# mdolab/dafoam

Hardware: NVIDIA H100
Metric: dRdWTPsi_GCells_per_s (higher is better)
Workload: dtype f64

## Files before the change

dafoam_b200/csrc/capi.cpp:

```cpp
#include "../../include/dab200.h"
#include "solver.hpp"
#include <cstring>
#include <string>

using namespace dab;

struct dab_solver
{
    Solver s;
};

static thread_local std::string g_err;
static dab_exchange_fn g_cbExchange = nullptr;
static dab_allreduce_fn g_cbAllreduce = nullptr;
static void* g_cbCtx = nullptr;

#define DAB_TRY try {
#define DAB_CATCH                                   \
    }                                               \
    catch (const std::exception& e)                 \
    {                                               \
        g_err = e.what();                           \
        return 1;                                   \
    }                                               \
// ... 587 lines not shown
        stats->pc_assemblies = s->s.kry.pcAssemblies;
        stats->n_matvec = st.nMatvec;
    }
    DAB_CATCH
}

int dab_solve_linear_eqn(dab_solver* s, const double* rhs, double* sol, int* fail, dab_ksp_stats* stats)
{
    DAB_TRY
    need(s, "solver");
    need(rhs, "rhs");
    need(sol, "sol");
    KspStats st;
    const int f = s->s.solveLinearEqn(rhs, sol, st);
    if (fail) *fail = f;
    if (stats)
    {
        stats->iterations = st.iterations;
        stats->converged_reason = st.reason;
        stats->initial_residual = st.r0;
        stats->final_residual = st.rn;
        stats->solve_seconds = st.solveSec;
        stats->pc_setup_seconds = st.pcSec;
        stats->pc_assemblies = s->s.kry.pcAssemblies;
        stats->n_matvec = st.nMatvec;
    }
    DAB_CATCH
}

int dab_calc_function(dab_solver* s, const char* name, double* value)
{
    DAB_TRY
    need(s, "solver");
    need(name, "name");
    need(value, "value");
    *value = s->s.calcFunction(name);
    DAB_CATCH
}

int dab_get_input_size(dab_solver* s, const char* name, const char* type, int64_t* out)
{
    DAB_TRY
    need(s, "solver");
    need(type, "type");
    (void)name;
    if (std::string(type) == "stateVar") *out = s->s.nDof();
    else if (std::string(type) == "patchVelocity") *out = 2;
    else if (std::string(type) == "volCoord") *out = (int64_t)s->s.hm.points.size();
    else if (std::string(type) == "patchVar") { need(name, "name"); *out = s->s.findPatchVar(name).nComp; }
    else if (std::string(type) == "fvSourcePar") { need(name, "name"); *out = (int64_t)s->s.findFvSourcePar(name).indices.size(); }
    else throw Error(std::string("getInputSize: unsupported input type ") + type);
    DAB_CATCH
}

int dab_get_output_size(dab_solver* s, const char* name, const char* type, int64_t* out)
{
    DAB_TRY
    need(s, "solver");
    need(type, "type");
    (void)name;
    const std::string t(type);
    if (t == "residual") *out = s->s.nDof();
    else if (t == "function") *out = 1;
    else throw Error("getOutputSize: unsupported output type " + t);
    DAB_CATCH
}

int dab_bench_set_vector(dab_solver* s, const double* x)
{
    DAB_TRY
    need(s, "solver");
    need(x, "x");
    s->s.be.h2d(s->s.dX.p, x, (size_t)s->s.nDof() * sizeof(double));
    DAB_CATCH
}

int dab_bench_device(dab_solver* s, int which, int n, double* ms_per_call, int64_t* kernel_launches)
{
    DAB_TRY
    need(s, "solver");
    need(ms_per_call, "ms_per_call");
    Solver& S = s->s;
    S.ensureRecorded();
    const long l0 = S.be.launches;
    auto t = S.be.timer();
    S.be.sync();
    t.start();
    for (int i = 0; i < n; i++)
    {
        switch (which)
        {
        case 0: S.matVecDev(S.dX.p, S.dY2.p); break;
        case 1: S.forward(0, S.dR.p); break;
        case 2: S.benchKernel(0); break;
        case 3: S.benchKernel(1); break;
        case 4: S.benchKernel(2); break;
        default: throw Error("dab_bench_device: unknown selector");
        }
    }
    *ms_per_call = t.stopMs() / (n > 0 ? n : 1);
    if (kernel_launches) *kernel_launches = S.be.launches - l0;
    DAB_CATCH
}

int dab_algorithmic_bytes(dab_solver* s, int which, int64_t* bytes)
{
    DAB_TRY
    need(s, "solver");
    need(bytes, "bytes");
    const HostMesh& m = s->s.hm;
    const int64_t nDof = s->s.nDof();
    const int64_t vecs = which == 0 ? 3 : 2;
    *bytes = 8 * vecs * nDof + (int64_t)m.nIF * (8 * 10 + 4 * 2) + (int64_t)m.nBF * (8 * 6 + 4 * 2) + (int64_t)m.nC * (8 * 5);
    DAB_CATCH
}

}
```

dafoam_b200/csrc/krylov.hpp:

```cpp
#pragma once
#include "backend.hpp"
#include "views.hpp"
#include "comm.hpp"
#include <atomic>
#include <cmath>
#include <thread>
#include <cstdint>
#include <vector>

namespace dab
{

struct KspStats
{
    int iterations = 0, reason = 0;
    double r0 = 0, rn = 0, solveSec = 0, pcSec = 0;
    int nMatvec = 0;
};

struct EllView
{
    int n;
    const int64_t* rowBase;
    const int32_t* rowStride;
// ... 55 lines not shown
        *q += eps * sc;
    }
};

struct FdFill
{
    EllView A;
    const int32_t* list;
    const int32_t* iperm;
    const int32_t* perm;
    const double *R0, *R1;
    double ieps;
    DAB_HD void operator()(int t) const
    {
        const int i = iperm[list[t]];
        const int64_t base = A.rowBase[i];
        const int64_t st = A.rowStride[i];
        const int len = A.rowLen[i];
        for (int e = 0; e < len; e++)
        {
            const int r = perm[A.col[base + e * st]];
            A.val[base + e * st] = (R1[r] - R0[r]) * ieps;
        }
    }
};

DAB_HD int ellFind(const EllView& A, int i, int j)
{
    const int64_t base = A.rowBase[i], st = A.rowStride[i];
    int lo = 0, hi = A.rowLen[i] - 1;
    while (lo <= hi)
    {
        const int mid = (lo + hi) >> 1;
        const int c = A.col[base + mid * st];
        if (c == j) return mid;
        if (c < j) lo = mid + 1;
        else hi = mid - 1;
    }
    return -1;
}

struct IluFactorColour
{
    EllView A;
    ColourView cv;
    double shift;
    DAB_HD void operator()(int t) const
    {
        for (int s = 0; s < cv.nSlots; s++)
        {
            if (t >= cv.slotCount[s]) break;
            const int i = cv.slotStart[s] + t;
            const int64_t bi = A.rowBase[i], si = A.rowStride[i];
            const int len = A.rowLen[i], di = A.diag[i];
            double rowMax = 0.0;
            for (int e = 0; e < len; e++)
            {
                const double v = fabs(A.val[bi + e * si]);
                rowMax = v > rowMax ? v : rowMax;
            }
            for (int e = 0; e < di; e++)
            {
                const int k = A.col[bi + e * si];
                const int64_t bk = A.rowBase[k], sk = A.rowStride[k];
                const int dk = A.diag[k], lk = A.rowLen[k];
                const double lik = A.val[bi + e * si] * A.val[bk + dk * sk];
                A.val[bi + e * si] = lik;
                if (lik == 0.0) continue;
                int pj = e + 1;
                for (int q = dk + 1; q < lk && pj < len; q++)
                {
                    const int j = A.col[bk + q * sk];
                    while (pj < len && A.col[bi + pj * si] < j) pj++;
                    if (pj < len && A.col[bi + pj * si] == j) A.val[bi + pj * si] -= lik * A.val[bk + q * sk];
                }
            }
            double d = A.val[bi + di * si];
            if (!(fabs(d) > shift * rowMax)) d = (d < 0.0 ? -1.0 : 1.0) * (rowMax > 0.0 ? shift * rowMax : 1.0);
            A.val[bi + di * si] = 1.0 / d;
        }
    }
};


template <int TRI_LANES>
DAB_HD double triRowDot(const EllView& A, int64_t bi, int64_t si, int e0, int e1, int lane, const double* y)
{
    double acc = 0.0;
    if (A.valF)
        for (int e = e0 + lane; e < e1; e += TRI_LANES) acc += (double)A.valF[bi + e * si] * y[A.col[bi + e * si]];
    else
        for (int e = e0 + lane; e < e1; e += TRI_LANES) acc += A.val[bi + e * si] * y[A.col[bi + e * si]];
    return acc;
}

template <int TRI_LANES>
struct TriLowerColour
{
    EllView A;
    ColourView cv;
    double* y;
    DAB_HD void operator()(int tt) const
    {
#if defined(__CUDA_ARCH__)
        const int t = tt / TRI_LANES, lane = tt - t * TRI_LANES;
        for (int s = 0; s < cv.nSlots; s++)
        {
            const bool on = t < cv.slotCount[s];
            const int i = cv.slotStart[s] + t;
            double acc = 0.0;
            if (on) acc = triRowDot<TRI_LANES>(A, cv.slotBase[s] + t, cv.slotCount[s], 0, A.diag[i], lane, y);
            for (int o = 1; o < TRI_LANES; o <<= 1) acc += __shfl_xor_sync(0xffffffffu, acc, o, TRI_LANES);
            if (on && lane == 0) y[i] -= acc;
            __syncwarp();
        }
#else
        if (tt % TRI_LANES) return;
        const int t = tt / TRI_LANES;
        for (int s = 0; s < cv.nSlots; s++)
        {
            if (t >= cv.slotCount[s]) break;
            const int i = cv.slotStart[s] + t;
            const int64_t bi = A.rowBase[i], si = A.rowStride[i];
            double part[TRI_LANES];
            for (int l = 0; l < TRI_LANES; l++) part[l] = triRowDot<TRI_LANES>(A, bi, si, 0, A.diag[i], l, y);
            for (int o = 1; o < TRI_LANES; o <<= 1)
                for (int l = 0; l < TRI_LANES; l++)
                    if (!(l & o)) part[l] += part[l | o];
            y[i] -= part[0];
        }
#endif
    }
};

template <int TRI_LANES>
struct TriUpperColour
{
    EllView A;
    ColourView cv;
    double* x;
    DAB_HD void operator()(int tt) const
    {
#if defined(__CUDA_ARCH__)
        const int t = tt / TRI_LANES, lane = tt - t * TRI_LANES;
        for (int s = cv.nSlots - 1; s >= 0; s--)
        {
            const bool on = t < cv.slotCount[s];
            const int i = cv.slotStart[s] + t;
            int64_t bi = 0, si = 0;
            int di = 0;
            double acc = 0.0;
            if (on)
            {
                bi = cv.slotBase[s] + t; si = cv.slotCount[s]; di = A.diag[i];
                acc = triRowDot<TRI_LANES>(A, bi, si, di + 1, A.rowLen[i], lane, x);
            }
            for (int o = 1; o < TRI_LANES; o <<= 1) acc += __shfl_xor_sync(0xffffffffu, acc, o, TRI_LANES);
            if (on && lane == 0) x[i] = (x[i] - acc) * (A.valF ? (double)A.valF[bi + di * si] : A.val[bi + di * si]);
            __syncwarp();
        }
#else
        if (tt % TRI_LANES) return;
        const int t = tt / TRI_LANES;
        for (int s = cv.nSlots - 1; s >= 0; s--)
        {
            if (t >= cv.slotCount[s]) continue;
            const int i = cv.slotStart[s] + t;
            const int64_t bi = A.rowBase[i], si = A.rowStride[i];
            const int di = A.diag[i];
            double part[TRI_LANES];
            for (int l = 0; l < TRI_LANES; l++) part[l] = triRowDot<TRI_LANES>(A, bi, si, di + 1, A.rowLen[i], l, x);
            for (int o = 1; o < TRI_LANES; o <<= 1)
                for (int l = 0; l < TRI_LANES; l++)
                    if (!(l & o)) part[l] += part[l | o];
            x[i] = (x[i] - part[0]) * (A.valF ? (double)A.valF[bi + di * si] : A.val[bi + di * si]);
        }
#endif
    }
};

DAB_HD double ellVal(const EllView& A, int64_t o) { return A.valF ? (double)A.valF[o] : A.val[o]; }

struct CvtToFloat
{
    const double* src;
    float* dst;
    DAB_HD void operator()(int i) const { dst[i] = (float)src[i]; }
};

struct GatherVec
{
    const double* src;
    const int32_t* idx;
    double* dst;
    DAB_HD void operator()(int i) const { dst[i] = src[idx[i]]; }
};
struct ScatterVec
{
    const double* src;
    const int32_t* idx;
    double* dst;
    DAB_HD void operator()(int i) const { dst[idx[i]] = src[i]; }
};
struct JacobiApply
{
    const double *src, *dinv;
    double* dst;
    DAB_HD void operator()(int i) const { dst[i] = src[i] * dinv[i]; }
};

struct MultiAxpy
{
    const double* V;
    int64_t ld;
    int k;
    const double* h;
    double* w;
    int assign;
    DAB_HD void operator()(int i) const
    {
        double s = 0.0;
        for (int j = 0; j < k; j++) s += h[j] * V[(int64_t)j * ld + i];
        w[i] = assign ? s : w[i] - s;
    }
};
struct ScaleCopy
{
    const double* src;
    double a;
    double* dst;
    DAB_HD void operator()(int i) const { dst[i] = a * src[i]; }
};
struct AxpyVec
{
    const double* x;
    double a;
    double* y;
    DAB_HD void operator()(int i) const { y[i] += a * x[i]; }
};
struct SubVec
{
    const double* b;
    double* r;
    DAB_HD void operator()(int i) const { r[i] = b[i] - r[i]; }
};

#ifndef DAB_HOSTSIM
constexpr int DOT_TILE = 8;
constexpr int DOT_BLOCKS = 132 * 4;
constexpr int DOT_THREADS = 256;
__global__ void __launch_bounds__(DOT_THREADS) multiDotPartial(const double* __restrict__ V, int64_t ld, int k, const double* __restrict__ w,
                                                               int n, double* __restrict__ partial)
{
    __shared__ double sm[DOT_THREADS / 32][DOT_TILE];
    const int lane = threadIdx.x & 31, warp = threadIdx.x >> 5;
    for (int j0 = 0; j0 < k; j0 += DOT_TILE)
    {
        const int nj = (k - j0) < DOT_TILE ? (k - j0) : DOT_TILE;
        double acc[DOT_TILE];
#pragma unroll
        for (int j = 0; j < DOT_TILE; j++) acc[j] = 0.0;
        for (int i = blockIdx.x * blockDim.x + threadIdx.x; i < n; i += gridDim.x * blockDim.x)
        {
            const double wi = w[i];
#pragma unroll
            for (int j = 0; j < DOT_TILE; j++)
                if (j < nj) acc[j] += V[(int64_t)(j0 + j) * ld + i] * wi;
        }
#pragma unroll
        for (int j = 0; j < DOT_TILE; j++)
        {
            double v = acc[j];
            for (int o = 16; o > 0; o >>= 1) v += __shfl_down_sync(0xffffffffu, v, o);
            if (lane == 0) sm[warp][j] = v;
        }
        __syncthreads();
        if (threadIdx.x < nj)
        {
            double v = 0.0;
            for (int q = 0; q < DOT_THREADS / 32; q++) v += sm[q][threadIdx.x];
            partial[(int64_t)blockIdx.x * k + j0 + threadIdx.x] = v;
        }
        __syncthreads();
    }
}
__global__ void multiDotFinal(const double* __restrict__ partial, int nb, int k, double* __restrict__ out)
// ... 382 lines not shown
```

dafoam_b200/csrc/launch_traits.hpp:

```cpp
#pragma once
#include "backend.hpp"
#include "fwd_kernels.hpp"
#include "rev_kernels.hpp"
#include "comp_kernels.hpp"
#include "comp_rev_kernels.hpp"
#include "primal_kernels.hpp"
#include "comp_primal_kernels.hpp"

namespace dab
{

#if !defined(DAB_HOSTSIM)
#ifndef DAB_REVB_MINBLOCKS
#define DAB_REVB_MINBLOCKS 2
#endif
#ifndef DAB_FWDB_MINBLOCKS
#define DAB_FWDB_MINBLOCKS 3
#endif
template <int NF, int FEAT> struct LaunchTraits<RevB<NF, FEAT>> { static constexpr int minBlocks = DAB_REVB_MINBLOCKS; };
template <int NF> struct LaunchTraits<RevA<NF>> { static constexpr int minBlocks = 5; };
template <int NF> struct LaunchTraits<RevC<NF>> { static constexpr int minBlocks = 4; };
template <int NF, int FEAT> struct LaunchTraits<FwdB<NF, FEAT>> { static constexpr int minBlocks = DAB_FWDB_MINBLOCKS; };
template <int NF, int FEAT> struct LaunchTraits<UEqnAssemble<NF, FEAT>> { static constexpr int minBlocks = DAB_FWDB_MINBLOCKS; };
template <int NF> struct LaunchTraits<NutEqnAssemble<NF>> { static constexpr int minBlocks = 4; };
template <int NF> struct LaunchTraits<cFwdB<NF>> { static constexpr int minBlocks = 2; };
template <int NF> struct LaunchTraits<cUEqnAssemble<NF>> { static constexpr int minBlocks = 2; };
template <int NF> struct LaunchTraits<cEEqnAssemble<NF>> { static constexpr int minBlocks = 3; };
template <int NF> struct LaunchTraits<cNutEqnAssemble<NF>> { static constexpr int minBlocks = 3; };
template <int NF> struct LaunchTraits<cPEqnAssemble<NF>> { static constexpr int minBlocks = 4; };
template <int NF> struct LaunchTraits<cPhiUpdate<NF>> { static constexpr int minBlocks = 4; };
#ifndef DAB_CREVA_MINBLOCKS
#define DAB_CREVA_MINBLOCKS 4
#endif
#ifndef DAB_CREVB_MINBLOCKS
#define DAB_CREVB_MINBLOCKS 3
#endif
#ifndef DAB_CREVE_MINBLOCKS
#define DAB_CREVE_MINBLOCKS 4
#endif
template <int NF> struct LaunchTraits<cRevB<NF>> { static constexpr int minBlocks = DAB_CREVB_MINBLOCKS; };
template <int NF> struct LaunchTraits<cRevA<NF>> { static constexpr int minBlocks = DAB_CREVA_MINBLOCKS; };
template <int NF> struct LaunchTraits<cRevE<NF>> { static constexpr int minBlocks = DAB_CREVE_MINBLOCKS; };
template <int NF> struct LaunchTraits<cRevC<NF>> { static constexpr int minBlocks = 4; };
template <int NF> struct LaunchTraits<cFwdE<NF>> { static constexpr int minBlocks = 4; };
template <int NF> struct LaunchTraits<cFwdC<NF>> { static constexpr int minBlocks = 4; };
#endif

}
```

dafoam_b200/csrc/solver.hpp:

```cpp
#pragma once
#include "backend.hpp"
#include "mesh.hpp"
#include "views.hpp"
#include "fwd_kernels.hpp"
#include "rev_kernels.hpp"
#include "tile_kernels.hpp"
#include "comp_kernels.hpp"
#include "comp_rev_kernels.hpp"
#include "krylov.hpp"
#include "primal_kernels.hpp"
#include "geom_kernels.hpp"
#include "comp_primal_kernels.hpp"
#include "launch_traits.hpp"
#include "partition.hpp"
#include "comm.hpp"
#include <chrono>
#include <cstdlib>
#include <cstdio>
#include <fstream>
#include <map>
#include <sys/stat.h>
#include <set>

namespace dab
// ... 2182 lines not shown
                    if (bj < 0) throw Error("writeSensMapSurface: no surface point within 9999999 of a wall point");
                    norm2 += best * best;
                    for (int k = 0; k < 3; k++) sens[(size_t)3 * (f - hm.nIF) + k] += dFdXs[3 * bj + k];
                }
                for (int k = 0; k < 3; k++) sens[(size_t)3 * (f - hm.nIF) + k] /= 3.0;
            }
        }
        const std::string dir = caseDirectory + "/" + timeName;
        ::mkdir(dir.c_str(), 0755);
        FILE* f = fopen((dir + "/" + name).c_str(), "w");
        if (!f) throw Error("cannot write " + dir + "/" + name);
        fprintf(f, "FoamFile\n{\n    version 2.0;\n    format ascii;\n    class volVectorField;\n    location \"%s\";\n    object %s;\n}\n\n"
                   "dimensions [0 0 0 0 0 0 0];\n\ninternalField uniform (0 0 0);\n\nboundaryField\n{\n", timeName.c_str(), name.c_str());
        for (size_t ip = 0; ip < hm.patches.size(); ip++)
        {
            const PatchDef& p = hm.patches[ip];
            fprintf(f, "    %s\n    {\n        type fixedValue;\n", p.name.c_str());
            if (hm.patchGeom[ip] == PG_WALL)
            {
                fprintf(f, "        value nonuniform List<vector> %d(", p.size);
                for (int i = 0; i < p.size; i++)
                {
                    const double* v = &sens[(size_t)3 * (p.start + i - hm.nIF)];
                    fprintf(f, "%s(%.17g %.17g %.17g)", i ? " " : "", v[0], v[1], v[2]);
                }
                fprintf(f, ");\n");
            }
            else
                fprintf(f, "        value uniform (0 0 0);\n");
            fprintf(f, "    }\n");
        }
        fprintf(f, "}\n");
        fclose(f);
        return std::sqrt(norm2);
    }

    void writeMeshPoints(const double* pts, const std::string& dirName) const
    {
        if (ghosted()) throw Error("mesh output needs an undecomposed mesh without cyclic patches in this build");
        const std::string d1 = caseDirectory + "/" + dirName, d2 = d1 + "/polyMesh";
        ::mkdir(d1.c_str(), 0755);
        ::mkdir(d2.c_str(), 0755);
        FILE* f = fopen((d2 + "/points").c_str(), "w");
        if (!f) throw Error("cannot write " + d2 + "/points");
        fprintf(f, "FoamFile\n{\n    version 2.0;\n    format ascii;\n    class vectorField;\n    location \"%s/polyMesh\";\n    object points;\n}\n\n%d\n(\n",
                dirName.c_str(), hm.nP);
        for (int i = 0; i < hm.nP; i++) fprintf(f, "(%.17g %.17g %.17g)\n", pts[3 * i], pts[3 * i + 1], pts[3 * i + 2]);
        fprintf(f, ")\n");
        fclose(f);
    }
    void readMeshPoints(const std::string& timeName)
    {
        std::vector<double> pts;
        readVectorField(caseDirectory + "/" + timeName + "/polyMesh/points", pts);
        if (pts.size() != hm.points.size()) throw Error("readMeshPoints: " + timeName + "/polyMesh/points has the wrong size");
        updateMesh(pts.data());
    }
    void readStateVars(const std::string& timeName) { initialStates(caseDirectory, timeName); }

    VolCoord volc;
    void uploadGeometry();
    void deviceGeometry();
    void downloadGeometry();
    void updateMesh(const double* pts);
    void volCoordSetup();
    void volCoordProduct(const double* psi, const FunctionDef* function, double seed, double* out);

    Primal primal;
    VecOps primalOps;
    void primalSetup();
    const double* primalSums(int k);
    void primalResidual(const EqnView& e, const double* x, const double* g, double* res);
    void primalJacobi(const EqnView& e, double* x, double* tmp, const double* g, const SegControl& ctl, double* res0);
    void primalCoarseSetup();
    void primalCoarseRefresh(const EqnView& e);
    void primalPrecond(const EqnView& e, const double* r, double* z);
    int primalPcg(const EqnView& e, double* x, const SegControl& ctl, double& res0);
    int solvePrimal(PrimalStats& st);

    void pcSymbolic();
    void calcPC();
    void applyPC(const double* v, double* z);
    void applyIlu(const double* v, double* z);
    void coarseSetup();
    void coarseRestrict(const double* v, bool toHost = true);
    int kspExtraMatvecs = 0;
    int solveLinearEqn(const double* rhs, double* sol, KspStats& st);
    int solveIdrs(const double* rhs, double* sol, KspStats& st);
    int solveFixedPoint(const double* rhs, double* sol, KspStats& st);
};

}

#include "solver_krylov.hpp"
#include "solver_primal.hpp"
#include "solver_volcoord.hpp"
```

dafoam_b200/csrc/solver_krylov.hpp:

```cpp
#pragma once
#include <algorithm>
#include <chrono>
#include <cstdio>

#include <memory>
#include <thread>

namespace dab
{

namespace detail
{
struct CellGraph
{
    int nC;
    std::vector<int> off, adj, stamp, queue;
    int tick = 0;
    void build(const HostMesh& m, const std::vector<int>* alias = nullptr)
    {
        nC = m.nC;
        auto cellOf = [&](int c) { return c < nC ? c : (alias ? (*alias)[c - nC] : -1); };
        off.assign(nC + 1, 0);
        for (int f = 0; f < m.nIF; f++)
        {
// ... 249 lines not shown
        auto within = [&](int lv) { return lv < 0 ? 0 : w.levelEnd[std::min(lv, (int)w.levelEnd.size() - 1)]; };
        for (int r = 0; r < ns; r++)
        {
            const int nIn = within(lvCell[ks][kindOf(r)]);
            for (int q = 0; q < nIn; q++)
            {
                const int x = w.cellsBall[q];
                if (blk > 0 && x / blk != c / blk) continue;
                cols.push_back(K.iperm[r < 3 ? 3 * x + r : r * nC + x]);
            }
        }
        w.faces.clear();
        const int nIn = within(lvPhiRes[ks]);
        for (int q = 0; q < nIn; q++) facesOf(w.cellsBall[q], w.faces);
        std::sort(w.faces.begin(), w.faces.end());
        w.faces.erase(std::unique(w.faces.begin(), w.faces.end()), w.faces.end());
        for (int f : w.faces)
            if (!(blk > 0 && blockCell(f) / blk != c / blk)) cols.push_back(K.iperm[offPhi + f]);
        std::sort(cols.begin(), cols.end());
    };
    auto faceRowCols = [&](Work& w, int f) {
        std::vector<int>& cols = w.cols;
        cols.clear();
        if (hm.own[f] >= nC)
        {
            cols.push_back(K.iperm[offPhi + f]);
            return;
        }
        int seeds[2];
        const int nSeeds = faceSeeds(f, seeds);
        G.ball(seeds, nSeeds, Lcf, w.cellsBall, w.sc, &w.levelEnd);
        for (int r = 0; r < ns; r++)
        {
            const int lv = lvOfPhi[kindOf(r)];
            const int nIn = lv < 0 ? 0 : w.levelEnd[std::min(lv, (int)w.levelEnd.size() - 1)];
            for (int q = 0; q < nIn; q++)
            {
                const int x = w.cellsBall[q];
                if (blk > 0 && x / blk != blockCell(f) / blk) continue;
                cols.push_back(K.iperm[r < 3 ? 3 * x + r : r * nC + x]);
            }
        }
        if (phiPhi)
        {
            w.faces.clear();
            for (int q = 0; q < nSeeds; q++) facesOf(seeds[q], w.faces);
            w.faces.push_back(f);
            std::sort(w.faces.begin(), w.faces.end());
            w.faces.erase(std::unique(w.faces.begin(), w.faces.end()), w.faces.end());
            for (int g : w.faces)
                if (g == f || !(blk > 0 && blockCell(g) / blk != blockCell(f) / blk)) cols.push_back(K.iperm[offPhi + g]);
        }
        else
            cols.push_back(K.iperm[offPhi + f]);
        std::sort(cols.begin(), cols.end());
    };
    detail::parallelFor(nC, nThreads, [&](int t, int b, int e) {
        Work& w = work[t];
        for (int c = b; c < e; c++)
        {
            cellBall(w, c);
            for (int s = 0; s < ns; s++)
            {
                if (s == 0 || s >= 3) cellRowCols(w, c, s);
                const int i = K.iperm[s < 3 ? 3 * c + s : s * nC + c];
                K.rowLen[i] = (int)w.cols.size();
                w.width[groupOfRow[i]] = std::max(w.width[groupOfRow[i]], (int)w.cols.size());
            }
        }
    });
    detail::parallelFor(nF, nThreads, [&](int t, int b, int e) {
        Work& w = work[t];
        for (int f = b; f < e; f++)
        {
            faceRowCols(w, f);
            const int i = K.iperm[offPhi + f];
            K.rowLen[i] = (int)w.cols.size();
            w.width[groupOfRow[i]] = std::max(w.width[groupOfRow[i]], (int)w.cols.size());
        }
    });
    lap("pattern: row lengths");
    for (const Work& w : work)
        for (int g = 0; g < nG; g++) width[g] = std::max(width[g], w.width[g]);
    std::vector<int64_t> gOff(nG + 1, 0);
    for (int g = 0; g < nG; g++) gOff[g + 1] = gOff[g] + (int64_t)width[g] * groupRows[g];
    K.ellSize = gOff[nG];
    {
        int g = 0;
        for (ColourView& cv : K.colours)
            for (int sl = 0; sl < cv.nSlots; sl++) cv.slotBase[sl] = gOff[g++];
    }
    K.rowBase.resize(K.n);
    K.rowStride.resize(K.n);
    K.diag.assign(K.n, -1);
    for (int i = 0; i < K.n; i++)
    {
        const int g = groupOfRow[i];
        K.rowBase[i] = gOff[g] + (i - groupStart[g]);
        K.rowStride[i] = groupRows[g];
    }
    std::unique_ptr<int32_t[]> hColOwned(new int32_t[(size_t)K.ellSize]);
    int32_t* hCol = hColOwned.get();
    K.nnz = 0;
    lap("pattern: ELL allocation");
    auto putRow = [&](Work& w, int i) {
        const std::vector<int>& cols = w.cols;
        for (size_t e = 0; e < cols.size(); e++)
        {
            hCol[(size_t)(K.rowBase[i] + (int64_t)e * K.rowStride[i])] = cols[e];
            if (cols[e] == i) K.diag[i] = (int)e;
        }
        for (int e = (int)cols.size(); e < width[groupOfRow[i]]; e++) hCol[(size_t)(K.rowBase[i] + (int64_t)e * K.rowStride[i])] = -1;
        w.nnz += (int64_t)cols.size();
        if (K.diag[i] < 0) throw Error("calcdRdWT: missing diagonal in the pattern");
    };
    detail::parallelFor(nC, nThreads, [&](int t, int b, int e) {
        Work& w = work[t];
        for (int c = b; c < e; c++)
        {
            cellBall(w, c);
            for (int s = 0; s < ns; s++)
            {
                if (s == 0 || s >= 3) cellRowCols(w, c, s);
                putRow(w, K.iperm[s < 3 ? 3 * c + s : s * nC + c]);
            }
        }
    });
    detail::parallelFor(nF, nThreads, [&](int t, int b, int e) {
        Work& w = work[t];
        for (int f = b; f < e; f++)
        {
            faceRowCols(w, f);
            putRow(w, K.iperm[offPhi + f]);
        }
    });
    for (const Work& w : work) K.nnz += w.nnz;
    lap("pattern: ELL fill");
    std::vector<int> fdCell;
    const int nFdCell = detail::greedyColour(nC, [&](int c, std::vector<int>& out) { G.ball(&c, 1, Lcc + 3, out); }, fdCell);
    std::vector<int> fdFace;
    std::vector<int> tmpCells;
    const int nFdFace = detail::greedyColour(nF, [&](int f, std::vector<int>& out) {
        int seeds[2];
        const int nSeeds = faceSeeds(f, seeds);
        G.ball(seeds, nSeeds, Lcf + 1, tmpCells);
        out.clear();
        for (int x : tmpCells) facesOf(x, out);
    }, fdFace);
    const int nFd = ns * nFdCell + nFdFace;
    std::vector<int> cnt(nFd + 1, 0);
    auto fdColourOf = [&](int ext) {
        if (ext < 3 * nC) return (ext % 3) * nFdCell + fdCell[ext / 3];
        if (ext < offPhi) return (ext / nC) * nFdCell + fdCell[ext % nC];
        return ns * nFdCell + fdFace[ext - offPhi];
    };
    for (int j = 0; j < K.n; j++) cnt[fdColourOf(j) + 1]++;
    for (int k = 0; k < nFd; k++) cnt[k + 1] += cnt[k];
    K.fdStart.assign(cnt.begin(), cnt.end());
    K.fdList.resize(K.n);
    {
        std::vector<int> pos(cnt.begin(), cnt.end() - 1);
        for (int j = 0; j < K.n; j++) K.fdList[pos[fdColourOf(j)]++] = j;
    }
    lap("perturbation colours");
    K.dPerm.upload(be, K.perm);
    K.dIPerm.upload(be, K.iperm);
// ... 318 lines not shown
            Cs.dApValSorted.upload(be, sVal);
            Cs.apValid = true;
            if (printInfo) fprintf(stderr, "[dab200] coarse space: sparse A*P with %llu entries (%.2f per row)\n", cnt, (double)cnt / n);
        }
        else if (printInfo)
            fprintf(stderr, "[dab200] coarse space: sparse A*P not usable (overflow or response outside the reach sets): matrix-free product kept\n");
        Cs.dApRow.release(); Cs.dApAgg.release(); Cs.dApVal.release();
    }
    Cs.factor(std::min(std::max(1, detail::hostThreads() / std::max(1, nRanks)), 32));
    {
        std::vector<double> invT;
        Cs.invertTransposed(invT, [&](int nItems, auto fn) {
            const int nt = nItems >= 256 ? std::max(1, detail::hostThreads() / std::max(1, nRanks)) : 1;
            if (nt == 1) fn(0, 0, nItems);
            else
            {
                std::vector<std::thread> th;
                for (int t = 0; t < nt; t++)
                    th.emplace_back([&, t]() { fn(t, (int)((int64_t)nItems * t / nt), (int)((int64_t)nItems * (t + 1) / nt)); });
                for (auto& x : th) x.join();
            }
        });
        Cs.dInvT.upload(be, invT);
    }
    Cs.valid = true;
    (void)offP;
}

inline void Solver::coarseRestrict(const double* v, bool toHost)
{
    Coarse& Cs = kry.coarse;
    const int offP = 3 * hm.nC;
    be.launch(Cs.nChunks, CoarseRestrict1{v + offP, Cs.dCells.p, Cs.dChunkStart.p, Cs.dPartial.p});
    be.zero(Cs.dRc.p, (size_t)Cs.nAggGlobal * sizeof(double));
    be.launch(Cs.nAggLocal, CoarseRestrict2{Cs.dPartial.p, Cs.dAggChunkOff.p, Cs.dRc.p + Cs.aggBase});
    comm.allreduceSum(be, Cs.dRc.p, Cs.nAggGlobal);
    if (toHost) be.d2h(Cs.hRc.data(), Cs.dRc.p, (size_t)Cs.nAggGlobal * sizeof(double));
}

inline void Solver::applyPC(const double* v, double* z)
{
    Krylov& K = kry;
    if (K.coarse.enabled && K.coarse.valid)
    {
        Coarse& Cs = K.coarse;
        const int n = nDof();
        coarseRestrict(v, false);
        be.launch(Cs.nAggGlobal, CoarseApply{Cs.dInvT.p, Cs.dRc.p, Cs.nAggGlobal, Cs.dYc.p});
        be.launch(n, CoarseProlong{Cs.dYc.p, Cs.dAggOf.p, 3 * hm.nC, hm.nC, Cs.aggBase, K.t2.p});
        if (Cs.apValid)
            be.launch(n, ApApply{Cs.dApPtr.p, Cs.dApAggSorted.p, Cs.dApValSorted.p, Cs.dYc.p, v, K.t3.p});
        else
        {
            matVecDev(K.t2.p, K.t3.p);
            kspExtraMatvecs++;
            be.launch(n, SubVec{v, K.t3.p});
        }
        applyIlu(K.t3.p, z);
        be.launch(n, AxpyVec{K.t2.p, 1.0, z});
    }
    else
        applyIlu(v, z);
    if (globalPCIters > 0)
    {
        const int n = nDof();
        if (K.t4.n < (size_t)n)
        {
            K.t4.alloc(be, n);
            K.t5.alloc(be, n);
        }
        for (int it = 0; it < globalPCIters; it++)
        {
            matVecDev(z, K.t4.p);
            kspExtraMatvecs++;
            be.launch(n, SubVec{v, K.t4.p});
            applyIlu(K.t4.p, K.t5.p);
            be.launch(n, AxpyVec{K.t5.p, richardsonOmega, z});
        }
    }
}

inline void Solver::applyIlu(const double* v, double* z)
{
    Krylov& K = kry;
    EllView A = K.view();
    be.launch(K.n, GatherVec{v, K.dPerm.p, K.t1.p});
    auto padded = [](int nCells, int lanes) { return (nCells * lanes + 31) / 32 * 32; };
    if (pcBlockCells > 0)
    {
        for (size_t k = 0; k < K.colours.size(); k++) be.launch(padded(K.colours[k].nCells, 4), TriLowerColour<4>{A, K.colours[k], K.t1.p});
        for (size_t k = K.colours.size(); k-- > 0;) be.launch(padded(K.colours[k].nCells, 4), TriUpperColour<4>{A, K.colours[k], K.t1.p});
    }
    else
    {
        for (size_t k = 0; k < K.colours.size(); k++) be.launch(padded(K.colours[k].nCells, 1), TriLowerColour<1>{A, K.colours[k], K.t1.p});
        for (size_t k = K.colours.size(); k-- > 0;) be.launch(padded(K.colours[k].nCells, 1), TriUpperColour<1>{A, K.colours[k], K.t1.p});
    }
    be.launch(K.n, ScatterVec{K.t1.p, K.dPerm.p, z});
}

inline int Solver::solveLinearEqn(const double* rhs, double* sol, KspStats& st)
{
    Krylov& K = kry;
    if (!K.pcValid && !(K.pcFactored && adjPCLag > 1 && K.symbolic)) calcPC();
    ensureRecorded();
    if (kspType == "idrs") return solveIdrs(rhs, sol, st);
    const int n = nDof();
    const int m = std::max(1, std::min(gmresRestart, gmresMaxIters));
    K.ops.init(be, &comm, m + 2);
    if (K.vCap < m + 1 || K.V.n < (size_t)(m + 1) * n)
    {
        K.V.alloc(be, (size_t)(m + 1) * n, false);
        K.vCap = m + 1;
        K.w.alloc(be, n);
        K.z.alloc(be, n);
        K.xdev.alloc(be, n);
        K.bdev.alloc(be, n);
        if (K.hdev.n < (size_t)(m + 2)) K.hdev.alloc(be, m + 2);
        K.ops.init(be, &comm, m + 2);
    }
    be.h2d(K.bdev.p, rhs, (size_t)n * sizeof(double));
    be.zero(K.xdev.p, (size_t)n * sizeof(double));
    auto timer = be.timer();
    be.sync();
    timer.start();
    const long l0 = be.launches;
    const double bnorm = K.ops.norm2(K.bdev.p, n);
    st.r0 = bnorm;
    st.nMatvec = 0;
    kspExtraMatvecs = 0;
    const double tol = std::max(gmresRelTol * bnorm, gmresAbsTol);
    std::vector<double> H((size_t)(m + 1) * m, 0.0), cs(m, 0.0), sn(m, 0.0), g(m + 1, 0.0), yv(m, 0.0), hcol(m + 2, 0.0);
    int its = 0, nRefine = 0, nTrueRestarts = 0;
    double rnorm = bnorm;
    int reason = 0;
    if (bnorm == 0.0)
    {
        reason = 3;
    }
    while (reason == 0)
    {
        double beta;
        if (its == 0)
        {
            be.d2d(K.w.p, K.bdev.p, (size_t)n * sizeof(double));
            beta = bnorm;
        }
        else
        {
            matVecDev(K.xdev.p, K.w.p);
            st.nMatvec++;
            be.launch(n, SubVec{K.bdev.p, K.w.p});
            beta = K.ops.norm2(K.w.p, n);
        }
        rnorm = beta;
        if (rnorm <= tol) { reason = rnorm <= gmresRelTol * bnorm ? 2 : 3; break; }
        be.launch(n, ScaleCopy{K.w.p, 1.0 / beta, K.V.p});
        std::fill(g.begin(), g.end(), 0.0);
        g[0] = beta;
        int k = 0;
        for (; k < m && its < gmresMaxIters; k++, its++)
        {
            double* vk = K.V.p + (size_t)k * n;
            double* vk1 = K.V.p + (size_t)(k + 1) * n;
            applyPC(vk, K.z.p);
            matVecDev(K.z.p, vk1);
            st.nMatvec++;
            const double* d = K.ops.dots(K.V.p, n, k + 2, vk1, n);
            for (int j = 0; j <= k; j++) hcol[j] = d[j];
            const double wn2 = d[k + 1];
            K.putCoeffs(be, hcol.data(), k + 1);
            be.launch(n, MultiAxpy{K.V.p, n, k + 1, K.hdev.p, vk1, 0});
            double hn2 = 0.0;
            for (int j = 0; j <= k; j++) hn2 += hcol[j] * hcol[j];
            double nrm;
            if (wn2 - hn2 < 0.25 * wn2 || useMGSO)
            {
                nRefine++;
                const double* d2 = K.ops.dots(K.V.p, n, k + 2, vk1, n);
                std::vector<double> h2(d2, d2 + k + 1);
                const double wn2b = d2[k + 1];
// ... 332 lines not shown
```

dafoam_b200/pyDASolvers.py:

```python
from __future__ import annotations

import ctypes as C
import json
import os
import time
import numpy as np

_HERE = os.path.dirname(os.path.abspath(__file__))
_LIBS = {}


class DAB200Error(RuntimeError):
    pass


class KspStats(C.Structure):
    _fields_ = [("iterations", C.c_int32), ("converged_reason", C.c_int32), ("initial_residual", C.c_double),
                ("final_residual", C.c_double), ("solve_seconds", C.c_double), ("pc_setup_seconds", C.c_double),
                ("n_matvec", C.c_int32), ("pc_assemblies", C.c_int32)]


class PrimalStats(C.Structure):
    _fields_ = [("iterations", C.c_int32), ("converged", C.c_int32), ("p_iterations", C.c_int32), ("reserved", C.c_int32),
                ("max_residual", C.c_double), ("res_u", C.c_double * 3), ("res_p", C.c_double), ("res_nutilda", C.c_double),
# ... 474 lines not shown

    def getPCMatrixSize(self):
        n, nnz = C.c_int64(), C.c_int64()
        self._raise(self._L.dab_get_pc_matrix(self._h, C.byref(n), C.byref(nnz), None, None, None))
        return int(n.value), int(nnz.value)

    def getPCMatrix(self):
        n, nnz = C.c_int64(), C.c_int64()
        self._raise(self._L.dab_get_pc_matrix(self._h, C.byref(n), C.byref(nnz), None, None, None))
        rp, cl, vl = np.zeros(n.value + 1, dtype=np.int64), np.zeros(nnz.value, dtype=np.int32), np.zeros(nnz.value)
        self._raise(self._L.dab_get_pc_matrix(self._h, C.byref(n), C.byref(nnz), rp.ctypes.data_as(C.POINTER(C.c_int64)),
                                              cl.ctypes.data_as(C.POINTER(C.c_int32)), _dp(vl)))
        return rp, cl[:nnz.value], vl[:nnz.value]

    def getPCFactors(self):
        n, nnz = C.c_int64(), C.c_int64()
        self._raise(self._L.dab_get_pc_factors(self._h, C.byref(n), C.byref(nnz), None, None, None, None, None))
        rp, cl, vl = np.zeros(n.value + 1, dtype=np.int64), np.zeros(nnz.value, dtype=np.int32), np.zeros(nnz.value)
        perm, colour = np.zeros(n.value, dtype=np.int32), np.zeros(n.value, dtype=np.int32)
        ip = C.POINTER(C.c_int32)
        self._raise(self._L.dab_get_pc_factors(self._h, C.byref(n), C.byref(nnz), rp.ctypes.data_as(C.POINTER(C.c_int64)),
                                               cl.ctypes.data_as(ip), _dp(vl), perm.ctypes.data_as(ip), colour.ctypes.data_as(ip)))
        return rp, cl[:nnz.value], vl[:nnz.value], perm, colour

    def getPCAggregates(self):
        agg = np.zeros(self.getNLocalCells(), dtype=np.int32)
        self._raise(self._L.dab_get_pc_aggregates(self._h, agg.ctypes.data_as(C.POINTER(C.c_int32))))
        return agg

    def initializedRdWTMatrixFree(self):
        return None

    def destroydRdWTMatrixFree(self):
        return None

    def createMLRKSPMatrixFree(self, jacPCMat, myKSP):
        assert jacPCMat.assembled, "call calcdRdWT(1, dRdWTPC) first"
        myKSP.ready = True

    def updateKSPPCMat(self, PCMat, myKSP):
        myKSP.ready = PCMat.assembled

    def solveLinearEqn(self, myKSP, rhsVec, solVec):
        n = self.getNLocalAdjointStates()
        _check_array(rhsVec, n, "rhs")
        _check_array(solVec, n, "sol")
        fail = C.c_int(1)
        st = KspStats()
        self._raise(self._L.dab_solve_linear_eqn(self._h, _dp(rhsVec), _dp(solVec), C.byref(fail), C.byref(st)))
        if myKSP is not None:
            myKSP.stats = st
        return int(fail.value)

    def applyPC(self, v, z):
        n = self.getNLocalAdjointStates()
        _check_array(v, n, "v")
        _check_array(z, n, "z")
        self._raise(self._L.dab_pc_apply(self._h, _dp(v), _dp(z)))

    def calcdRdWTPsiAD(self, psi, dRdWTPsi):
        n = self.getNLocalAdjointStates()
        _check_array(psi, n, "psi")
        _check_array(dRdWTPsi, n, "dRdWTPsi")
        self._raise(self._L.dab_drdwt_mat_vec(self._h, _dp(psi), _dp(dRdWTPsi)))

    def solveAdjoint(self, dFdW, psi):
        ksp = KSP()
        return self.solveLinearEqn(ksp, dFdW, psi), ksp.stats

    def benchDevice(self, which, n):
        ms = C.c_double()
        nl = C.c_int64()
        self._raise(self._L.dab_bench_device(self._h, C.c_int(which), C.c_int(n), C.byref(ms), C.byref(nl)))
        return float(ms.value), int(nl.value)

    def benchSetVector(self, x):
        _check_array(x, self.getNLocalAdjointStates(), "x")
        self._raise(self._L.dab_bench_set_vector(self._h, _dp(x)))

    def algorithmicBytes(self, which=0):
        v = C.c_int64()
        self._raise(self._L.dab_algorithmic_bytes(self._h, C.c_int(which), C.byref(v)))
        return int(v.value)
```

include/dab200.h:

```cpp
#ifndef DAB200_H
#define DAB200_H

#include <stdint.h>

#ifdef __cplusplus
extern "C" {
#endif

typedef struct dab_solver dab_solver;

enum dab_bc_kind
{
    DAB_BC_FIXED_VALUE = 0,
    DAB_BC_ZERO_GRADIENT = 1,
    DAB_BC_INLET_OUTLET = 2,
    DAB_BC_OUTLET_INLET = 3,
    DAB_BC_SYMMETRY = 4,
    DAB_BC_CALCULATED = 5,
    DAB_BC_NUT_LOW_RE = 6
};

typedef struct dab_ksp_stats
{
    int32_t iterations;
// ... 23 lines not shown
const char* dab_version(void);

int dab_create(const char* case_dir, const char* args_all, const char* options_json, int device, int rank,
               int n_ranks, const void* nccl_unique_id, dab_solver** out);
int dab_destroy(dab_solver* s);

int dab_nccl_unique_id(void* out128);

int dab_get_local_to_global(dab_solver* s, int what, int64_t* out);

typedef void (*dab_exchange_cb)(void* ctx, int n_peers, const int* peers, const double* const* send_bufs, const int* send_counts,
                                double* const* recv_bufs, const int* recv_counts);
typedef void (*dab_allreduce_cb)(void* ctx, double* buf, int n);
int dab_set_comm_callbacks(dab_exchange_cb exchange, dab_allreduce_cb allreduce, void* ctx);

int dab_n_local_adjoint_states(dab_solver* s, int64_t* out);
int dab_n_local_cells(dab_solver* s, int64_t* out);
int dab_n_global_cells(dab_solver* s, int64_t* out);
int dab_n_local_points(dab_solver* s, int64_t* out);
int dab_volcoord_evaluations(dab_solver* s, int64_t* out);
int dab_n_local_faces(dab_solver* s, int64_t* out);
int dab_n_local_internal_faces(dab_solver* s, int64_t* out);

int dab_update_options(dab_solver* s, const char* options_json);

int dab_update_of_fields(dab_solver* s, const double* states);
int dab_get_of_fields(dab_solver* s, double* states);

int dab_get_of_mesh_points(dab_solver* s, double* points);
int dab_write_adjoint_fields(dab_solver* s, const char* function, double write_time, const double* psi);
int dab_write_fields(dab_solver* s, double write_time);

int dab_read_state_vars(dab_solver* s, double time_val);
int dab_read_mesh_points(dab_solver* s, double time_val);
int dab_write_mesh_points(dab_solver* s, const double* points, const char* dir_name);
int dab_write_sens_map_surface(dab_solver* s, const char* name, const double* dfdxs, const double* xs, int size, double time_name,
                               double* min_distance_norm);
int dab_write_sens_map_field(dab_solver* s, const char* name, const double* dfdfield, const char* field_type, double time_name);
#define DAB_CHECK_MESH_REPORT 11
int dab_check_mesh(dab_solver* s, double max_non_orth, double max_skewness, double max_aspect_ratio, int max_incorrectly_oriented_faces,
                   int* mesh_ok, double* report);

int dab_update_of_mesh(dab_solver* s, const double* points);
int dab_get_of_field(dab_solver* s, const char* name, const char* type, double* field);

int dab_get_residuals(dab_solver* s, int is_pc, double* residuals);

int dab_calc_jac_t_vec_product(dab_solver* s, const char* input_name, const char* input_type, const double* input,
                               const char* output_name, const char* output_type, const double* seed,
                               double* product);

int dab_drdwt_mat_vec(dab_solver* s, const double* x, double* y);

int dab_calc_drdwt_pc(dab_solver* s);

int dab_pc_apply(dab_solver* s, const double* v, double* z);

int dab_solve_linear_eqn(dab_solver* s, const double* rhs, double* sol, int* fail, dab_ksp_stats* stats);

int dab_run_fp_adj(dab_solver* s, const double* dfdw, double* psi, int* fail, dab_ksp_stats* stats);

int dab_get_pc_matrix(dab_solver* s, int64_t* n_rows, int64_t* nnz, int64_t* row_ptr, int32_t* cols, double* vals);

int dab_get_pc_factors(dab_solver* s, int64_t* n_rows, int64_t* nnz, int64_t* row_ptr, int32_t* cols, double* vals, int32_t* perm,
                       int32_t* colour);

int dab_get_pc_aggregates(dab_solver* s, int32_t* agg_of);

int dab_calc_pc_mat_fvmatrix(dab_solver* s, int turb_only, int64_t* nnz, int32_t* rows, int32_t* cols, double* vals);

int dab_set_solver_input(dab_solver* s, const char* input_name, const char* input_type, int input_size, const double* inputs,
                         const double* seeds);

int dab_solve_primal(dab_solver* s, int* fail, dab_primal_stats* stats);

int dab_calc_function(dab_solver* s, const char* name, double* value);

int dab_get_input_size(dab_solver* s, const char* name, const char* type, int64_t* out);
int dab_get_output_size(dab_solver* s, const char* name, const char* type, int64_t* out);

int dab_bench_device(dab_solver* s, int which, int n, double* ms_per_call, int64_t* kernel_launches);
int dab_bench_set_vector(dab_solver* s, const double* x);
int dab_algorithmic_bytes(dab_solver* s, int which, int64_t* bytes);

#ifdef __cplusplus
}
#endif
#endif
```

Before: 1.267.

## Fuse ILU permutation into triangular solves and batch row loads

The separate gather and scatter kernels around the ILU triangular solves are removed. The permutation is now folded into the lower solve, which reads the rhs through perm, and the upper solve, which writes z through perm. The row dot product is templated on value type and batches column and value loads with streaming loads ahead of the y gathers to expose memory-level parallelism. Per-slot diag and rowLen are hoisted into registers, with rowLen packed into 16 bits. Launch-bounds minBlocks is set for the triangular kernels, and benchmarking and layout APIs are added.

```diff
diff --git a/dafoam_b200/csrc/capi.cpp b/dafoam_b200/csrc/capi.cpp
--- a/dafoam_b200/csrc/capi.cpp
+++ b/dafoam_b200/csrc/capi.cpp
@@ -693,6 +693,7 @@
     need(ms_per_call, "ms_per_call");
     Solver& S = s->s;
     S.ensureRecorded();
+    if (which >= 5 && !S.kry.pcFactored) throw Error("dab_bench_device: selectors 5-8 time the preconditioner; assemble it first (calcdRdWT)");
     const long l0 = S.be.launches;
     auto t = S.be.timer();
     S.be.sync();
@@ -706,6 +707,10 @@
         case 2: S.benchKernel(0); break;
         case 3: S.benchKernel(1); break;
         case 4: S.benchKernel(2); break;
+        case 5: S.applyPC(S.dX.p, S.dY2.p); break;
+        case 6: S.applyIlu(S.dX.p, S.dY2.p); break;
+        case 7: S.iluLower(S.dX.p); break;
+        case 8: S.iluUpper(S.dY2.p); break;
         default: throw Error("dab_bench_device: unknown selector");
         }
     }
@@ -726,4 +731,34 @@
     DAB_CATCH
 }
 
-}
+int dab_pc_algorithmic_bytes(dab_solver* s, int which, int64_t* bytes)
+{
+    DAB_TRY
+    need(s, "solver");
+    need(bytes, "bytes");
+    if (!s->s.kry.symbolic) throw Error("dab_pc_algorithmic_bytes: no preconditioner pattern yet (calcdRdWT)");
+    *bytes = s->s.pcAlgorithmicBytes(which);
+    DAB_CATCH
+}
+
+int dab_pc_layout(dab_solver* s, int cap, int* n_colours, int64_t* rows_per_colour, int64_t* cells_per_colour, int64_t* nnz)
+{
+    DAB_TRY
+    need(s, "solver");
+    need(n_colours, "n_colours");
+    const Krylov& K = s->s.kry;
+    if (!K.symbolic) throw Error("dab_pc_layout: no preconditioner pattern yet (calcdRdWT)");
+    *n_colours = (int)K.colours.size();
+    for (int k = 0; k < (int)K.colours.size() && k < cap; k++)
+    {
+        const ColourView& cv = K.colours[k];
+        int64_t rows = 0;
+        for (int sl = 0; sl < cv.nSlots; sl++) rows += cv.slotCount[sl];
+        if (rows_per_colour) rows_per_colour[k] = rows;
+        if (cells_per_colour) cells_per_colour[k] = cv.nCells;
+    }
+    if (nnz) *nnz = K.nnz;
+    DAB_CATCH
+}
+
+}
diff --git a/dafoam_b200/csrc/krylov.hpp b/dafoam_b200/csrc/krylov.hpp
--- a/dafoam_b200/csrc/krylov.hpp
+++ b/dafoam_b200/csrc/krylov.hpp
@@ -161,36 +161,85 @@
     }
 };
 
-
-template <int TRI_LANES>
-DAB_HD double triRowDot(const EllView& A, int64_t bi, int64_t si, int e0, int e1, int lane, const double* y)
+#ifndef DAB_TRI_BATCH
+#define DAB_TRI_BATCH 16
+#endif
+template <class FT>
+constexpr int TRI_BATCH = sizeof(FT) == 4 ? DAB_TRI_BATCH : DAB_TRI_BATCH / 2;
+
+#if defined(__CUDA_ARCH__)
+template <int TRI_LANES, class FT>
+__device__ __forceinline__ void triBatch(double& acc, const FT* val, const int32_t* col, int64_t o, int64_t step, int nb, const double* y)
+{
+    constexpr int B = TRI_BATCH<FT>;
+    int c[B];
+    FT v[B];
+    double x[B];
+#pragma unroll
+    for (int b = 0; b < B; b++)
+        if (b < nb)
+        {
+            c[b] = __ldcs(col + o + b * step);
+            v[b] = __ldcs(val + o + b * step);
+        }
+#pragma unroll
+    for (int b = 0; b < B; b++)
+        if (b < nb) x[b] = y[c[b]];
+#pragma unroll
+    for (int b = 0; b < B; b++)
+        if (b < nb) acc += (double)v[b] * x[b];
+}
+#endif
+
+template <int TRI_LANES, class FT>
+DAB_HD double triRowDot(const FT* val, const int32_t* col, int64_t bi, int64_t si, int e0, int e1, int lane, const double* y)
 {
     double acc = 0.0;
-    if (A.valF)
-        for (int e = e0 + lane; e < e1; e += TRI_LANES) acc += (double)A.valF[bi + e * si] * y[A.col[bi + e * si]];
-    else
-        for (int e = e0 + lane; e < e1; e += TRI_LANES) acc += A.val[bi + e * si] * y[A.col[bi + e * si]];
+#if defined(__CUDA_ARCH__)
+    const int64_t step = (int64_t)TRI_LANES * si;
+    int64_t o = bi + (int64_t)(e0 + lane) * si;
+    constexpr int B = TRI_BATCH<FT>;
+    int e = e0 + lane;
+    for (; e + (B - 1) * TRI_LANES < e1; e += B * TRI_LANES, o += B * step)
+        triBatch<TRI_LANES>(acc, val, col, o, step, B, y);
+    if (e < e1) triBatch<TRI_LANES>(acc, val, col, o, step, (e1 - e + TRI_LANES - 1) / TRI_LANES, y);
+#else
+    for (int e = e0 + lane; e < e1; e += TRI_LANES) acc += (double)val[bi + e * si] * y[col[bi + e * si]];
+#endif
     return acc;
 }
 
-template <int TRI_LANES>
+template <int TRI_LANES, class FT>
 struct TriLowerColour
 {
     EllView A;
+    const FT* fv;
     ColourView cv;
+    const double* v;
+    const int32_t* perm;
     double* y;
     DAB_HD void operator()(int tt) const
     {
 #if defined(__CUDA_ARCH__)
         const int t = tt / TRI_LANES, lane = tt - t * TRI_LANES;
-        for (int s = 0; s < cv.nSlots; s++)
-        {
+        int dg[MAXSLOT];
+#pragma unroll
+        for (int s = 0; s < MAXSLOT; s++)
+            dg[s] = s < cv.nSlots && t < cv.slotCount[s] ? A.diag[cv.slotStart[s] + t] : 0;
+#pragma unroll
+        for (int s = 0; s < MAXSLOT; s++)
+        {
+            if (s >= cv.nSlots) break;
             const bool on = t < cv.slotCount[s];
             const int i = cv.slotStart[s] + t;
-            double acc = 0.0;
-            if (on) acc = triRowDot<TRI_LANES>(A, cv.slotBase[s] + t, cv.slotCount[s], 0, A.diag[i], lane, y);
+            double rhs = 0.0, acc = 0.0;
+            if (on)
+            {
+                if (lane == 0) rhs = v[perm[i]];
+                acc = triRowDot<TRI_LANES>(fv, A.col, cv.slotBase[s] + t, cv.slotCount[s], 0, dg[s], lane, y);
+            }
             for (int o = 1; o < TRI_LANES; o <<= 1) acc += __shfl_xor_sync(0xffffffffu, acc, o, TRI_LANES);
-            if (on && lane == 0) y[i] -= acc;
+            if (on && lane == 0) y[i] = rhs - acc;
             __syncwarp();
         }
 #else
@@ -202,40 +251,61 @@
             const int i = cv.slotStart[s] + t;
             const int64_t bi = A.rowBase[i], si = A.rowStride[i];
             double part[TRI_LANES];
-            for (int l = 0; l < TRI_LANES; l++) part[l] = triRowDot<TRI_LANES>(A, bi, si, 0, A.diag[i], l, y);
+            for (int l = 0; l < TRI_LANES; l++) part[l] = triRowDot<TRI_LANES>(fv, A.col, bi, si, 0, A.diag[i], l, y);
             for (int o = 1; o < TRI_LANES; o <<= 1)
                 for (int l = 0; l < TRI_LANES; l++)
                     if (!(l & o)) part[l] += part[l | o];
-            y[i] -= part[0];
-        }
-#endif
-    }
-};
-
-template <int TRI_LANES>
+            y[i] = v[perm[i]] - part[0];
+        }
+#endif
+    }
+};
+
+template <int TRI_LANES, class FT>
 struct TriUpperColour
 {
     EllView A;
+    const FT* fv;
     ColourView cv;
+    const int32_t* perm;
     double* x;
+    double* z;
     DAB_HD void operator()(int tt) const
     {
 #if defined(__CUDA_ARCH__)
         const int t = tt / TRI_LANES, lane = tt - t * TRI_LANES;
-        for (int s = cv.nSlots - 1; s >= 0; s--)
-        {
+        int rg[MAXSLOT];
+#pragma unroll
+        for (int s = 0; s < MAXSLOT; s++)
+        {
+            const int i = cv.slotStart[s] + t;
+            rg[s] = s < cv.nSlots && t < cv.slotCount[s] ? A.diag[i] | A.rowLen[i] << 16 : 0;
+        }
+#pragma unroll
+        for (int s = MAXSLOT - 1; s >= 0; s--)
+        {
+            if (s >= cv.nSlots) continue;
             const bool on = t < cv.slotCount[s];
             const int i = cv.slotStart[s] + t;
-            int64_t bi = 0, si = 0;
-            int di = 0;
-            double acc = 0.0;
+            const int di = rg[s] & 0xffff;
+            const int64_t bi = cv.slotBase[s] + t, si = cv.slotCount[s];
+            double acc = 0.0, xi = 0.0, dinv = 0.0;
             if (on)
             {
-                bi = cv.slotBase[s] + t; si = cv.slotCount[s]; di = A.diag[i];
-                acc = triRowDot<TRI_LANES>(A, bi, si, di + 1, A.rowLen[i], lane, x);
+                if (lane == 0)
+                {
+                    xi = x[i];
+                    dinv = (double)fv[bi + di * si];
+                }
+                acc = triRowDot<TRI_LANES>(fv, A.col, bi, si, di + 1, rg[s] >> 16, lane, x);
             }
             for (int o = 1; o < TRI_LANES; o <<= 1) acc += __shfl_xor_sync(0xffffffffu, acc, o, TRI_LANES);
-            if (on && lane == 0) x[i] = (x[i] - acc) * (A.valF ? (double)A.valF[bi + di * si] : A.val[bi + di * si]);
+            if (on && lane == 0)
+            {
+                const double r = (xi - acc) * dinv;
+                x[i] = r;
+                z[perm[i]] = r;
+            }
             __syncwarp();
         }
 #else
@@ -248,11 +318,12 @@
             const int64_t bi = A.rowBase[i], si = A.rowStride[i];
             const int di = A.diag[i];
             double part[TRI_LANES];
-            for (int l = 0; l < TRI_LANES; l++) part[l] = triRowDot<TRI_LANES>(A, bi, si, di + 1, A.rowLen[i], l, x);
+            for (int l = 0; l < TRI_LANES; l++) part[l] = triRowDot<TRI_LANES>(fv, A.col, bi, si, di + 1, A.rowLen[i], l, x);
             for (int o = 1; o < TRI_LANES; o <<= 1)
                 for (int l = 0; l < TRI_LANES; l++)
                     if (!(l & o)) part[l] += part[l | o];
-            x[i] = (x[i] - part[0]) * (A.valF ? (double)A.valF[bi + di * si] : A.val[bi + di * si]);
+            x[i] = (x[i] - part[0]) * (double)fv[bi + di * si];
+            z[perm[i]] = x[i];
         }
 #endif
     }
@@ -267,20 +338,6 @@
     DAB_HD void operator()(int i) const { dst[i] = (float)src[i]; }
 };
 
-struct GatherVec
-{
-    const double* src;
-    const int32_t* idx;
-    double* dst;
-    DAB_HD void operator()(int i) const { dst[i] = src[idx[i]]; }
-};
-struct ScatterVec
-{
-    const double* src;
-    const int32_t* idx;
-    double* dst;
-    DAB_HD void operator()(int i) const { dst[idx[i]] = src[i]; }
-};
 struct JacobiApply
 {
     const double *src, *dinv;
diff --git a/dafoam_b200/csrc/launch_traits.hpp b/dafoam_b200/csrc/launch_traits.hpp
--- a/dafoam_b200/csrc/launch_traits.hpp
+++ b/dafoam_b200/csrc/launch_traits.hpp
@@ -6,6 +6,7 @@
 #include "comp_rev_kernels.hpp"
 #include "primal_kernels.hpp"
 #include "comp_primal_kernels.hpp"
+#include "krylov.hpp"
 
 namespace dab
 {
@@ -44,6 +45,11 @@
 template <int NF> struct LaunchTraits<cRevC<NF>> { static constexpr int minBlocks = 4; };
 template <int NF> struct LaunchTraits<cFwdE<NF>> { static constexpr int minBlocks = 4; };
 template <int NF> struct LaunchTraits<cFwdC<NF>> { static constexpr int minBlocks = 4; };
+#ifndef DAB_TRI_MINBLOCKS
+#define DAB_TRI_MINBLOCKS 4
+#endif
+template <int L, class FT> struct LaunchTraits<TriLowerColour<L, FT>> { static constexpr int minBlocks = DAB_TRI_MINBLOCKS; };
+template <int L, class FT> struct LaunchTraits<TriUpperColour<L, FT>> { static constexpr int minBlocks = DAB_TRI_MINBLOCKS; };
 #endif
 
 }
diff --git a/dafoam_b200/csrc/solver.hpp b/dafoam_b200/csrc/solver.hpp
--- a/dafoam_b200/csrc/solver.hpp
+++ b/dafoam_b200/csrc/solver.hpp
@@ -2288,6 +2288,9 @@
     void calcPC();
     void applyPC(const double* v, double* z);
     void applyIlu(const double* v, double* z);
+    void iluLower(const double* v);
+    void iluUpper(double* z);
+    int64_t pcAlgorithmicBytes(int which) const;
     void coarseSetup();
     void coarseRestrict(const double* v, bool toHost = true);
     int kspExtraMatvecs = 0;
diff --git a/dafoam_b200/csrc/solver_krylov.hpp b/dafoam_b200/csrc/solver_krylov.hpp
--- a/dafoam_b200/csrc/solver_krylov.hpp
+++ b/dafoam_b200/csrc/solver_krylov.hpp
@@ -355,6 +355,8 @@
     lap("pattern: row lengths");
     for (const Work& w : work)
         for (int g = 0; g < nG; g++) width[g] = std::max(width[g], w.width[g]);
+    for (int g = 0; g < nG; g++)
+        if (width[g] >= 1 << 15) throw Error("calcdRdWT: a row of dRdWTPC longer than the 16-bit field TriUpperColour packs it in");
     std::vector<int64_t> gOff(nG + 1, 0);
     for (int g = 0; g < nG; g++) gOff[g + 1] = gOff[g] + (int64_t)width[g] * groupRows[g];
     K.ellSize = gOff[nG];
@@ -839,21 +841,58 @@
 
 inline void Solver::applyIlu(const double* v, double* z)
 {
+    iluLower(v);
+    iluUpper(z);
+}
+
+static inline int triPadded(int nCells, int lanes) { return (nCells * lanes + 31) / 32 * 32; }
+
+template <class FT>
+static void launchIluLower(Backend& be, const Krylov& K, const EllView& A, const FT* fv, int lanes, const double* v)
+{
+    for (const ColourView& cv : K.colours)
+        if (lanes == 4) be.launch(triPadded(cv.nCells, 4), TriLowerColour<4, FT>{A, fv, cv, v, K.dPerm.p, K.t1.p});
+        else be.launch(triPadded(cv.nCells, 1), TriLowerColour<1, FT>{A, fv, cv, v, K.dPerm.p, K.t1.p});
+}
+
+template <class FT>
+static void launchIluUpper(Backend& be, const Krylov& K, const EllView& A, const FT* fv, int lanes, double* z)
+{
+    for (size_t k = K.colours.size(); k-- > 0;)
+        if (lanes == 4) be.launch(triPadded(K.colours[k].nCells, 4), TriUpperColour<4, FT>{A, fv, K.colours[k], K.dPerm.p, K.t1.p, z});
+        else be.launch(triPadded(K.colours[k].nCells, 1), TriUpperColour<1, FT>{A, fv, K.colours[k], K.dPerm.p, K.t1.p, z});
+}
+
+inline void Solver::iluLower(const double* v)
+{
     Krylov& K = kry;
-    EllView A = K.view();
-    be.launch(K.n, GatherVec{v, K.dPerm.p, K.t1.p});
-    auto padded = [](int nCells, int lanes) { return (nCells * lanes + 31) / 32 * 32; };
-    if (pcBlockCells > 0)
-    {
-        for (size_t k = 0; k < K.colours.size(); k++) be.launch(padded(K.colours[k].nCells, 4), TriLowerColour<4>{A, K.colours[k], K.t1.p});
-        for (size_t k = K.colours.size(); k-- > 0;) be.launch(padded(K.colours[k].nCells, 4), TriUpperColour<4>{A, K.colours[k], K.t1.p});
-    }
-    else
-    {
-        for (size_t k = 0; k < K.colours.size(); k++) be.launch(padded(K.colours[k].nCells, 1), TriLowerColour<1>{A, K.colours[k], K.t1.p});
-        for (size_t k = K.colours.size(); k-- > 0;) be.launch(padded(K.colours[k].nCells, 1), TriUpperColour<1>{A, K.colours[k], K.t1.p});
-    }
-    be.launch(K.n, ScatterVec{K.t1.p, K.dPerm.p, z});
+    const EllView A = K.view();
+    const int lanes = pcBlockCells > 0 ? 4 : 1;
+    if (A.valF) launchIluLower(be, K, A, A.valF, lanes, v);
+    else launchIluLower<double>(be, K, A, A.val, lanes, v);
+}
+
+inline void Solver::iluUpper(double* z)
+{
+    Krylov& K = kry;
+    const EllView A = K.view();
+    const int lanes = pcBlockCells > 0 ? 4 : 1;
+    if (A.valF) launchIluUpper(be, K, A, A.valF, lanes, z);
+    else launchIluUpper<double>(be, K, A, A.val, lanes, z);
+}
+
+inline int64_t Solver::pcAlgorithmicBytes(int which) const
+{
+    const Krylov& K = kry;
+    const int64_t bv = K.useF32 ? 4 : 8, n = K.n;
+    int64_t lower = 0, upper = 0;
+    for (int i = 0; i < K.n; i++)
+    {
+        lower += K.diag[i];
+        upper += K.rowLen[i] - K.diag[i];
+    }
+    const int64_t bl = lower * (bv + 4) + 8 * n + 16 * n, bu = upper * (bv + 4) + 12 * n + 24 * n;
+    return which == 1 ? bl : which == 2 ? bu : bl + bu;
 }
 
 inline int Solver::solveLinearEqn(const double* rhs, double* sol, KspStats& st)
diff --git a/dafoam_b200/pyDASolvers.py b/dafoam_b200/pyDASolvers.py
--- a/dafoam_b200/pyDASolvers.py
+++ b/dafoam_b200/pyDASolvers.py
@@ -580,3 +580,17 @@
         v = C.c_int64()
         self._raise(self._L.dab_algorithmic_bytes(self._h, C.c_int(which), C.byref(v)))
         return int(v.value)
+
+    def pcAlgorithmicBytes(self, which=0):
+        v = C.c_int64()
+        self._raise(self._L.dab_pc_algorithmic_bytes(self._h, C.c_int(which), C.byref(v)))
+        return int(v.value)
+
+    def pcLayout(self):
+        nc = C.c_int()
+        self._raise(self._L.dab_pc_layout(self._h, C.c_int(0), C.byref(nc), None, None, None))
+        rows = (C.c_int64 * max(nc.value, 1))()
+        cells = (C.c_int64 * max(nc.value, 1))()
+        nnz = C.c_int64()
+        self._raise(self._L.dab_pc_layout(self._h, nc, C.byref(nc), rows, cells, C.byref(nnz)))
+        return [int(r) for r in rows[:nc.value]], [int(c) for c in cells[:nc.value]], int(nnz.value)
diff --git a/include/dab200.h b/include/dab200.h
--- a/include/dab200.h
+++ b/include/dab200.h
@@ -129,6 +129,8 @@
 int dab_bench_device(dab_solver* s, int which, int n, double* ms_per_call, int64_t* kernel_launches);
 int dab_bench_set_vector(dab_solver* s, const double* x);
 int dab_algorithmic_bytes(dab_solver* s, int which, int64_t* bytes);
+int dab_pc_algorithmic_bytes(dab_solver* s, int which, int64_t* bytes);
+int dab_pc_layout(dab_solver* s, int cap, int* n_colours, int64_t* rows_per_colour, int64_t* cells_per_colour, int64_t* nnz);
 
 #ifdef __cplusplus
 }
```

Result: no change. 1.268 (median of 6 runs) (+0.1%).
